# earthspecies/avex

Measured on AMD Instinct MI355X. Metric: clips/s (10 s @ 16 kHz) embedding extraction, BEATs-base, higher is better.
Workload: dtype f16; 1 GPU; BEATs-base (12L/768/3072/12H, 90.7 M params, synthetic weights), batch 256 x 10 s @ 16 kHz per GPU, wav resident in HBM -> mean-pooled 768-d embedding; global_batch=256, samples_per_clip=160000, parallelism=dp1, world_size=1, inputs=avex_amd.synth.noise_clips(seed=0), keyed by global clip index, chunk_clips=256, streams=1, residual_stream=half, layernorm_fold=True

## Files before the change

### avex_amd/csrc/attention16.hip

```cpp
#include <stdlib.h>

#include "common.h"
#include "attention_plan.h"

namespace {

typedef int a3_i32x2 __attribute__((ext_vector_type(2)));
typedef int a3_i32x4 __attribute__((ext_vector_type(4)));
template <int N> struct a3_ic { static constexpr int value = N; };
template <typename T> struct a3_v2;
template <> struct a3_v2<_Float16> { typedef _Float16 type __attribute__((ext_vector_type(2))); };
template <> struct a3_v2<__bf16> { typedef __bf16 type __attribute__((ext_vector_type(2))); };

constexpr int A3_TMAX = 512;
constexpr int A3_KBUF = 32768;
constexpr int A3_HALF = 65536;
constexpr int A3_TPAD = 64;
constexpr int A3_TLD = A3_TPAD + 1040;
constexpr int A3_TAB_OFF = 2 * A3_HALF;
constexpr int A3X_KBUF = 9 * 4096;
constexpr int A3X_HALF = 2 * A3X_KBUF;
constexpr int A3X_KN = 544;
constexpr int A3X_KADD_OFF = 2 * A3X_HALF;
constexpr int A3X_GW_OFF = A3X_KADD_OFF + 2 * A3X_KN * 4;
constexpr int ATT3X_LDS = A3X_GW_OFF + 136 * 4;
constexpr int A3_TAB_BYTES = 4 * A3_TLD * 4;
constexpr int A3_KADD_OFF = A3_TAB_OFF + A3_TAB_BYTES;
constexpr int A3_GW_OFF = A3_KADD_OFF + 2 * A3_TMAX * 4;
constexpr int ATT3_LDS = A3_GW_OFF + 136 * 4;
constexpr float A3_THR = 8.f;
constexpr float A3_SUM_HI = 4096.f;
constexpr float A3_SUM_LO = 0.015625f;

#ifndef A3_KO
#define A3_KO 0
#endif
#ifndef A3_STAMPS
#define A3_STAMPS 0
#endif
#if A3_STAMPS
__device__ unsigned long long g_a3_stamps[3 * 16 * 8 * 16 * 16];
#endif

static __device__ __forceinline__ float a3_rows_sum(float x) {
    const unsigned u = __builtin_bit_cast(unsigned, x);
    const auto r = __builtin_amdgcn_permlane16_swap(u, u, false, false);
    const float y = __builtin_bit_cast(float, (unsigned)r[0]) + __builtin_bit_cast(float, (unsigned)r[1]);
    const unsigned v = __builtin_bit_cast(unsigned, y);
    const auto q = __builtin_amdgcn_permlane32_swap(v, v, false, false);
    return __builtin_bit_cast(float, (unsigned)q[0]) + __builtin_bit_cast(float, (unsigned)q[1]);
}
static __device__ __forceinline__ float a3_rows_max(float x) {
    const unsigned u = __builtin_bit_cast(unsigned, x);
    const auto r = __builtin_amdgcn_permlane16_swap(u, u, false, false);
    const float y = fmaxf(__builtin_bit_cast(float, (unsigned)r[0]), __builtin_bit_cast(float, (unsigned)r[1]));
    const unsigned v = __builtin_bit_cast(unsigned, y);
    const auto q = __builtin_amdgcn_permlane32_swap(v, v, false, false);
    return fmaxf(__builtin_bit_cast(float, (unsigned)q[0]), __builtin_bit_cast(float, (unsigned)q[1]));
}

static __device__ __forceinline__ void a3_dma16(const void* src, const char* lds_dst) {
    const unsigned lds = (unsigned)(__UINTPTR_TYPE__)(__attribute__((address_space(3))) const char*)lds_dst;
    asm volatile("s_mov_b32 m0, %1\n\tglobal_load_lds_dwordx4 %0, off" ::"v"(src), "s"(lds) : "memory");
}

template <typename T, bool BIAS, bool XT = false>
__global__ __launch_bounds__(512) void attention3_kernel(const T* __restrict__ qkv, int Tn, int Tq, int H, int Bc, int per_block,
                                                        const float* __restrict__ bias_tab, const float* __restrict__ grep_w,
                                                        const float* __restrict__ grep_b, const float* __restrict__ grep_a,
                                                        const uint8_t* __restrict__ key_pad, T* __restrict__ out, int q_log2e) {
    extern __shared__ __attribute__((aligned(16))) char smem[];
    typedef typename Half<T>::v8 v8;
    typedef typename Half<T>::v4 v4;
    static_assert(!XT || !BIAS, "the nine-tile last phase takes the bias table's LDS");
    constexpr int NB = 4, NW = 8, NT = 512, NKT = XT ? 9 : 8;
    constexpr int KBUF = XT ? A3X_KBUF : A3_KBUF, HALF = XT ? A3X_HALF : A3_HALF, KN = XT ? A3X_KN : A3_TMAX;
    float* tab = (float*)(smem + A3_TAB_OFF);
    float* kadd = (float*)(smem + (XT ? A3X_KADD_OFF : A3_KADD_OFF));
    T* gwh = (T*)(smem + (XT ? A3X_GW_OFF : A3_GW_OFF));
    float* gwb = (float*)(smem + (XT ? A3X_GW_OFF : A3_GW_OFF) + 512);

    const int tid = threadIdx.x, lane = tid & 63;
    const int wave = __builtin_amdgcn_readfirstlane(tid >> 6);
    const int c = lane & 15, g = lane >> 4;
    const int n_units = Bc * H;
    const int w0 = blockIdx.x * per_block;
    const int w1 = w0 + per_block < n_units ? w0 + per_block : n_units;
    if (w0 >= w1) return;
    const int E = H * 64;
    const int64_t ld = 3 * (int64_t)E;
    const float NEG_INF = -__builtin_inff();
    const int nh = Tn > 256 ? 2 : 1;
    const int np = (w1 - w0) * nh;
    const int nkt = (Tn + 31) >> 5;
    const int Q0 = 64 * wave;
    const bool has_q = Q0 < Tq;

    int h_cur = w0 / Bc, b_cur = w0 - h_cur * Bc;
    int half = 0;
    int h_ld = h_cur, b_ld = b_cur, half_ld = 0;
    int item_par = 0;

    auto dma_piece = [&](int ph, int u) __attribute__((always_inline)) {
        const T* base = qkv + (int64_t)b_ld * Tn * ld + h_ld * 64;
        char* buf = smem + (ph & 1) * HALF;
        int lane = tid & 63;
        asm volatile("" : "+v"(lane));
        const int ri = 4 * wave + u;
        const int kl = 8 * ri + (lane >> 3);
        int key = half_ld * 256 + kl;
        key = key < Tn ? key : Tn - 1;
        const int chunk = (lane & 7) ^ ((kl >> 1) & 7);
        a3_dma16(base + (int64_t)key * ld + E + chunk * 8, buf + ri * 1024);
        int vkey = half_ld * 256 + 8 * ri + ((lane >> 1) & 7);
        vkey = vkey < Tn ? vkey : Tn - 1;
        a3_dma16(base + (int64_t)vkey * ld + 2 * E + 16 * (lane >> 4) + 8 * (lane & 1), buf + KBUF + ri * 1024);
        if (XT && u == 3 && half_ld == nh - 1 && wave < 4) {
            const int rx = 32 + wave;
            const int klx = 8 * rx + (lane >> 3);
            int kx = half_ld * 256 + klx;
            kx = kx < Tn ? kx : Tn - 1;
            a3_dma16(base + (int64_t)kx * ld + E + ((lane & 7) ^ ((klx >> 1) & 7)) * 8, buf + rx * 1024);
            int vx = half_ld * 256 + 8 * rx + ((lane >> 1) & 7);
            vx = vx < Tn ? vx : Tn - 1;
            a3_dma16(base + (int64_t)vx * ld + 2 * E + 16 * (lane >> 4) + 8 * (lane & 1), buf + KBUF + rx * 1024);
        }
    };
    auto dma_advance = [&]() __attribute__((always_inline)) {
        if (++half_ld == nh) { half_ld = 0; if (++b_ld == Bc) { b_ld = 0; ++h_ld; } }
    };
    auto write_kadd = [&](int slot, int b) __attribute__((always_inline)) {
        for (int j = tid; j < KN; j += NT) {
            bool ok = j < Tn;
            if (ok && key_pad) ok = key_pad[(int64_t)b * Tn + j] == 0;
            kadd[slot * KN + j] = ok ? 0.f : NEG_INF;
        }
    };

    v8 qf[NB][2];
    auto load_q = [&](int h, int b) __attribute__((always_inline)) {
        const T* base = qkv + (int64_t)b * Tn * ld + h * 64;
        int lane = tid & 63;
        asm volatile("" : "+v"(lane));
        const int c = lane & 15, g = lane >> 4;
#pragma unroll
        for (int nb = 0; nb < NB; ++nb) {
            int q = Q0 + 16 * nb + c;
            q = q < Tq ? q : Tq - 1;
            const T* src = base + (int64_t)q * ld + 8 * g;
            asm volatile("global_load_dwordx4 %0, %2, off\n\tglobal_load_dwordx4 %1, %2, off offset:64" : "=&v"(qf[nb][0]), "=&v"(qf[nb][1]) : "v"(src) : "memory");
        }
    };
    if (wave >= NW / 2) __builtin_amdgcn_s_setprio(1);
    load_q(h_cur, b_cur);
#pragma unroll
    for (int u = 0; u < 4; ++u) dma_piece(0, u);
    dma_advance();
    write_kadd(0, b_cur);
    if (tid < 64) {
        float a = 0.f, bb = 0.f;
        if (grep_w) {
            a = (grep_w[0 * 64 + tid] + grep_w[1 * 64 + tid]) + (grep_w[2 * 64 + tid] + grep_w[3 * 64 + tid]);
            bb = (grep_w[4 * 64 + tid] + grep_w[5 * 64 + tid]) + (grep_w[6 * 64 + tid] + grep_w[7 * 64 + tid]);
        }
        const float wsc = 8.0f * 0.6931471805599453f;
        const float wa = a * wsc, wb = bb * wsc;
        const T wah = (T)wa, wbh = (T)wb;
        gwh[0 * 64 + tid] = wah; gwh[1 * 64 + tid] = wbh;
        gwh[2 * 64 + tid] = (T)(wa - (float)wah); gwh[3 * 64 + tid] = (T)(wb - (float)wbh);
        if (tid == 0) {
            gwb[0] = grep_w ? (grep_b[0] + grep_b[1]) + (grep_b[2] + grep_b[3]) : 0.f;
            gwb[1] = grep_w ? (grep_b[4] + grep_b[5]) + (grep_b[6] + grep_b[7]) : 0.f;
        }
    }
    if (tid < 4 * A3_TPAD) tab[(tid >> 6) * A3_TLD + (tid & 63)] = 0.f;

    int h_tab = -1;
    f32x2 gm[NB];
    float l_run[NB];
    unsigned long long refm[NB];
    f32x4 o[NB][4];
#pragma unroll
    for (int nb = 0; nb < NB; ++nb) {
        gm[nb] = (f32x2){1.f, 0.f}; l_run[nb] = 0.f; refm[nb] = 0ull;
#pragma unroll
        for (int db = 0; db < 4; ++db) o[nb][db] = (f32x4){0.f, 0.f, 0.f, 0.f};
    }
    const int v_lane = 1024 * (g >> 1) + 128 * (g & 1) + 32 * (c >> 2) + 8 * (c & 3);
    const float cs = q_log2e ? 0.125f : 0.125f * 1.4426950408889634f;

    int n_st = 0;
    auto store_item = [&](int h, int b) __attribute__((always_inline)) {
        n_st = 0;
        if (!has_q) return;
        int lane = tid & 63;
        asm volatile("" : "+v"(lane));
        const int c = lane & 15, g = lane >> 4;
#pragma unroll
        for (int nb = 0; nb < NB; ++nb) n_st += Q0 + 16 * nb < Tq ? 2 : 0;
#pragma unroll
        for (int nb = 0; nb < NB; ++nb) {
            if (Q0 + 16 * nb >= Tq) continue;
            const float l_tot = a3_rows_sum(l_run[nb]);
            const float inv = __builtin_amdgcn_rcpf(l_tot);
            const f32x2 inv2 = {inv, inv};
            typedef typename a3_v2<T>::type v2;
            auto pk = [&](const f32x4 v, int hi) __attribute__((always_inline)) -> unsigned {
                const f32x2 x = (f32x2){v[2 * hi], v[2 * hi + 1]} * inv2;
                const v2 h = {(T)x[0], (T)x[1]};
                unsigned u = __builtin_bit_cast(unsigned, h);
                asm volatile("" : "+v"(u));
                return u;
            };
            int w[2][4];
#pragma unroll
            for (int p = 0; p < 2; ++p) {
                const auto s0 = __builtin_amdgcn_permlane16_swap(pk(o[nb][2 * p], 0), pk(o[nb][2 * p + 1], 0), false, false);
                const auto s1 = __builtin_amdgcn_permlane16_swap(pk(o[nb][2 * p], 1), pk(o[nb][2 * p + 1], 1), false, false);
                w[p][0] = (int)s0[0]; w[p][1] = (int)s1[0]; w[p][2] = (int)s0[1]; w[p][3] = (int)s1[1];
            }
            const int qrow = Q0 + 16 * nb + c;
            T* orow = out + ((int64_t)b * Tn + qrow) * E + h * 64 + 16 * (g & 1) + 8 * (g >> 1);
#pragma unroll
            for (int p = 0; p < 2; ++p) {
                const a3_i32x4 wv = {w[p][0], w[p][1], w[p][2], w[p][3]};
                if (qrow < Tq) *(a3_i32x4*)(orow + 32 * p) = wv;
            }
        }
    };

    for (int ph = 0; ph < np; ++ph) {
        const bool last_half = half == nh - 1;
        const bool more_items = ph + (nh - half) < np;
#define A3_PT(i) if (A3_STAMPS) { __builtin_amdgcn_sched_barrier(0); pt[i] = __builtin_amdgcn_s_memtime(); __builtin_amdgcn_sched_barrier(0); }
        unsigned long long pt[16];
        if (A3_STAMPS) { for (int i = 0; i < 16; ++i) pt[i] = 0; pt[15] = __builtin_amdgcn_s_memrealtime(); }
        A3_PT(0)
        {
            const int nwait = (half == 0 && ph > 0) ? n_st : 0;
            asm volatile("s_cmp_eq_u32 %8, 8\n\ts_cbranch_scc1 1f\n\t"
                         "s_cmp_eq_u32 %8, 6\n\ts_cbranch_scc1 2f\n\t"
                         "s_cmp_eq_u32 %8, 4\n\ts_cbranch_scc1 3f\n\t"
                         "s_cmp_eq_u32 %8, 2\n\ts_cbranch_scc1 4f\n\t"
                         "s_waitcnt vmcnt(0) lgkmcnt(0)\n\ts_branch 5f\n"
                         "1:\n\ts_waitcnt vmcnt(8) lgkmcnt(0)\n\ts_branch 5f\n"
                         "2:\n\ts_waitcnt vmcnt(6) lgkmcnt(0)\n\ts_branch 5f\n"
                         "3:\n\ts_waitcnt vmcnt(4) lgkmcnt(0)\n\ts_branch 5f\n"
                         "4:\n\ts_waitcnt vmcnt(2) lgkmcnt(0)\n"
                         "5:"
                         : "+v"(qf[0][0]), "+v"(qf[0][1]), "+v"(qf[1][0]), "+v"(qf[1][1]), "+v"(qf[2][0]), "+v"(qf[2][1]), "+v"(qf[3][0]), "+v"(qf[3][1])
                         : "s"(nwait)
                         : "scc", "memory");
        }
        __builtin_amdgcn_s_barrier();
        A3_PT(1)
        if (half == 0) {
            if (BIAS && h_cur != h_tab) {
                for (int r = tid; r < 1040; r += NT) {
                    float v = 0.f;
                    if (r < 2 * Tn - 1) v = bias_tab[(int64_t)h_cur * (2 * Tn - 1) + r] * 1.4426950408889634f;
#pragma unroll
                    for (int sft = 0; sft < 4; ++sft)
                        if (r - sft >= 0) tab[sft * A3_TLD + A3_TPAD + (r - sft)] = v;
                }
                h_tab = h_cur;
                __syncthreads();
            }
            if (more_items) {
                int bn = b_cur + 1;
                bn = bn == Bc ? 0 : bn;
                write_kadd(item_par ^ 1, bn);
            }
            const T qs = (T)cs;
#pragma unroll
            for (int nb = 0; nb < NB; ++nb)
#pragma unroll
                for (int s = 0; s < 2; ++s)
#pragma unroll
                    for (int e8 = 0; e8 < 8; ++e8) qf[nb][s][e8] = qf[nb][s][e8] * qs;
            if (grep_w) {
                const v8 gA0 = *(const v8*)(gwh + (c & 3) * 64 + 8 * g), gA1 = *(const v8*)(gwh + (c & 3) * 64 + 32 + 8 * g);
                const float ba = gwb[0], bb = gwb[1], ah = grep_a[h_cur];
#pragma unroll
                for (int nb = 0; nb < NB; ++nb) {
                    f32x4 acc = mfma16(gA0, qf[nb][0], (f32x4){0.f, 0.f, 0.f, 0.f});
                    acc = mfma16(gA1, qf[nb][1], acc);
                    const float sa = (acc[0] + acc[2]) + ba, sb = (acc[1] + acc[3]) + bb;
                    const float ga = __builtin_amdgcn_rcpf(1.f + __expf(-sa)), gb = __builtin_amdgcn_rcpf(1.f + __expf(-sb));
                    gm[nb][0] = ga * (gb * ah - 1.f) + 2.f;
                }
            } else {
#pragma unroll
                for (int nb = 0; nb < NB; ++nb) gm[nb][0] = 1.f;
            }
        }
        const bool do_dma = ph + 1 < np;
        int dma_done = 0;
        A3_PT(2)
        if (has_q) {
            const char* Kb = smem + (ph & 1) * HALF;
            const float* kad = kadd + item_par * KN + half * 256 + 4 * g;
            const int kt_lim = (XT && last_half) ? 9 : 8;
            int kt_end = nkt - half * 8 < kt_lim ? nkt - half * 8 : kt_lim;
            const char* kp[2];
#pragma unroll
            for (int s = 0; s < 2; ++s) kp[s] = Kb + c * 128 + (((4 * s + g) ^ ((c >> 1) & 7)) << 4);
            const int e0 = 4 * g - (Q0 + c) + (Tn - 1) + 256 * half;
            const float* tp = tab + (e0 & 3) * A3_TLD + A3_TPAD + (e0 & ~3);
            const unsigned vaddr = (unsigned)(__UINTPTR_TYPE__)(__attribute__((address_space(3))) const char*)(Kb + KBUF + v_lane);

            v8 kf[2][2];
#pragma unroll
            for (int s = 0; s < 2; ++s)
#pragma unroll
                for (int kb = 0; kb < 2; ++kb) kf[s][kb] = *(const v8*)(kp[s] + 2048 * kb);
            f32x4 run[5];
            f32x4 Sq[NB][2];
            auto masked_at = [&](int ktl) __attribute__((always_inline)) { return key_pad != nullptr || (half * 8 + ktl) * 32 + 32 > Tn; };
            auto acc_start = [&](int nb, int kb, const f32x4 t4) __attribute__((always_inline)) {
                const f32x2 ta = {t4[0], t4[1]}, tb = {t4[2], t4[3]};
                f32x2 ea, eb;
                asm("v_pk_fma_f32 %0, %1, %2, %1 op_sel:[0,0,1] op_sel_hi:[0,1,1] neg_lo:[0,0,1] neg_hi:[0,0,1]" : "=v"(ea) : "v"(gm[nb]), "v"(ta));
                asm("v_pk_fma_f32 %0, %1, %2, %1 op_sel:[0,0,1] op_sel_hi:[0,1,1] neg_lo:[0,0,1] neg_hi:[0,0,1]" : "=v"(eb) : "v"(gm[nb]), "v"(tb));
                Sq[nb][kb] = (f32x4){ea[0], ea[1], eb[0], eb[1]};
            };
            auto acc_plain = [&](int nb) __attribute__((always_inline)) {
                const float nm = -gm[nb][1];
                Sq[nb][0] = (f32x4){nm, nm, nm, nm};
                Sq[nb][1] = (f32x4){nm, nm, nm, nm};
            };
            auto mask_acc = [&](int ktl) __attribute__((always_inline)) {
                const f32x4 k0 = *(const f32x4*)(kad + 32 * ktl), k1 = *(const f32x4*)(kad + 32 * ktl + 16);
#pragma unroll
                for (int nb = 0; nb < NB; ++nb) { Sq[nb][0] += k0; Sq[nb][1] += k1; }
            };
            if (BIAS) {
#pragma unroll
                for (int w = -3; w <= 1; ++w) run[w + 3] = *(const f32x4*)(tp + 16 * w);
#pragma unroll
                for (int nb = 0; nb < NB; ++nb)
#pragma unroll
                    for (int kb = 0; kb < 2; ++kb) acc_start(nb, kb, run[kb - nb + 3]);
            } else {
#pragma unroll
                for (int nb = 0; nb < NB; ++nb) acc_plain(nb);
            }
            if (masked_at(0)) mask_acc(0);
#define A3_FENCE() do { if (!(A3_KO & 32)) __builtin_amdgcn_sched_barrier(0); } while (0)
            auto tile = [&](auto KT) __attribute__((always_inline)) {
                constexpr int kt = decltype(KT)::value;
                typedef typename a3_v2<T>::type v2;
                a3_i32x2 vt[2][4];
                f32x2 pp[NB][4];
                unsigned pfw[NB][4];
                f32x2 lsa[NB], lsb[NB];
                float sum[NB];
                unsigned long long badm[NB];
                auto E = [&](int nb, int i) __attribute__((always_inline)) {
                    const int kb = i >> 1, r = 2 * (i & 1);
                    if (A3_KO & 2) { pp[nb][i] = (f32x2){Sq[nb][kb][r], Sq[nb][kb][r + 1]}; return; }
                    float x0 = Sq[nb][kb][r], x1 = Sq[nb][kb][r + 1];
                    asm volatile("" : "+v"(x0), "+v"(x1));
                    Sq[nb][kb][r] = x0; Sq[nb][kb][r + 1] = x1;
                    pp[nb][i] = (f32x2){__builtin_amdgcn_exp2f(x0), __builtin_amdgcn_exp2f(x1)};
                };
                auto cvt2 = [&](const f32x2 x) __attribute__((always_inline)) -> unsigned {
                    const v2 h = {(T)x[0], (T)x[1]};
                    unsigned u = __builtin_bit_cast(unsigned, h);
                    asm volatile("" : "+v"(u));
                    return u;
                };
                auto X = [&](int nb, int i) __attribute__((always_inline)) {
                    if (i == 0) { pfw[nb][0] = cvt2(pp[nb][0]); pfw[nb][1] = cvt2(pp[nb][1]); lsa[nb] = pp[nb][0] + pp[nb][1]; }
                    if (i == 1) { pfw[nb][2] = cvt2(pp[nb][2]); pfw[nb][3] = cvt2(pp[nb][3]); lsb[nb] = pp[nb][2] + pp[nb][3]; }
                    if (i == 2) { lsa[nb] += lsb[nb]; sum[nb] = hsum2(lsa[nb]); }
                    if (i == 3) {
                        badm[nb] = __builtin_amdgcn_ballot_w64(!(sum[nb] < A3_SUM_HI)) | (__builtin_amdgcn_ballot_w64(!(sum[nb] >= A3_SUM_LO)) & ~refm[nb]);
                    }
                };
                auto redo = [&](int nb) __attribute__((always_inline)) {
                    float mx = fmaxf(fmaxf(fmaxf(Sq[nb][0][0], Sq[nb][0][1]), fmaxf(Sq[nb][0][2], Sq[nb][0][3])),
                                     fmaxf(fmaxf(Sq[nb][1][0], Sq[nb][1][1]), fmaxf(Sq[nb][1][2], Sq[nb][1][3])));
                    mx = a3_rows_max(mx);
                    const bool rs = (refm[nb] >> lane) & 1ull;
                    const bool need = rs ? mx > A3_THR : mx != NEG_INF;
                    const float d = need ? mx : 0.f;
                    const float alpha = (need && rs) ? __builtin_amdgcn_exp2f(-d) : 1.f;
                    refm[nb] |= __builtin_amdgcn_ballot_w64(need);
                    gm[nb][1] += d;
                    l_run[nb] *= alpha;
#pragma unroll
                    for (int db = 0; db < 4; ++db) o[nb][db] *= alpha;
                    f32x2 ls = {0.f, 0.f};
#pragma unroll
                    for (int i = 0; i < 4; ++i) {
                        const int kb = i >> 1, r = 2 * (i & 1);
                        const f32x2 q2 = {__builtin_amdgcn_exp2f(Sq[nb][kb][r] - d), __builtin_amdgcn_exp2f(Sq[nb][kb][r + 1] - d)};
                        ls += q2;
                        const v2 h = {(T)q2[0], (T)q2[1]};
                        pfw[nb][i] = __builtin_bit_cast(unsigned, h);
                    }
                    sum[nb] = hsum2(ls);
                };
                auto check = [&](int nb) __attribute__((always_inline)) {
                    if (A3_KO & 1) { }
                    else if (__builtin_expect(badm[nb] != 0ull, 0)) redo(nb);
                    else refm[nb] = ~0ull;
                    l_run[nb] += sum[nb];
                };
                auto pfrag = [&](int nb) __attribute__((always_inline)) -> v8 {
                    typedef unsigned a3_u32x4 __attribute__((ext_vector_type(4)));
                    const a3_u32x4 w = {pfw[nb][0], pfw[nb][1], pfw[nb][2], pfw[nb][3]};
                    return __builtin_bit_cast(v8, w);
                };
                auto acc_next = [&](int j) __attribute__((always_inline)) {
                    if (kt + 1 >= NKT) return;
                    const int nn = j >> 1, kb = j & 1;
                    if ((A3_KO & 16) || !BIAS) { if (kb == 0) acc_plain(nn); }
                    else acc_start(nn, kb, run[(2 * (kt + 1) + kb - nn + 3) % 5]);
                };
#define A3_TS(i) if (A3_STAMPS == 2 && (kt == 6 || kt == 1)) { __builtin_amdgcn_sched_barrier(0); ts[i] = __builtin_amdgcn_s_memtime(); __builtin_amdgcn_sched_barrier(0); }
                unsigned long long ts[12];
                A3_TS(0)
#pragma unroll
                for (int i = 0; i < 4; ++i) {
                    const int s = i >> 1, kb = i & 1;
                    if (!(A3_KO & 4)) Sq[0][kb] = mfma16(kf[s][kb], qf[0][s], Sq[0][kb]);
                    A3_FENCE();
                }
                if (kt < 4 && do_dma) { dma_piece(ph + 1, kt); dma_done = kt + 1; A3_FENCE(); }
                {
#define A3_TR(dst, OFF) asm volatile("ds_read_b64_tr_b16 %0, %1 offset:%2" : "=v"(dst) : "v"(vaddr), "n"(OFF))
                    A3_TR(vt[0][0], 4096 * kt + 0);    A3_TR(vt[1][0], 4096 * kt + 2048 + 0);
                    A3_TR(vt[0][1], 4096 * kt + 256);  A3_TR(vt[1][1], 4096 * kt + 2048 + 256);
                    A3_TR(vt[0][2], 4096 * kt + 512);  A3_TR(vt[1][2], 4096 * kt + 2048 + 512);
                    A3_TR(vt[0][3], 4096 * kt + 768);  A3_TR(vt[1][3], 4096 * kt + 2048 + 768);
#undef A3_TR
                    if (BIAS && kt + 1 < NKT) {
                        run[(2 * kt + 5) % 5] = *(const f32x4*)(tp + 16 * (2 * kt + 2));
                        run[(2 * kt + 6) % 5] = *(const f32x4*)(tp + 16 * (2 * kt + 3));
                    }
                    A3_FENCE();
                }
                A3_TS(1)
#pragma unroll
                for (int nb = 1; nb < NB; ++nb) {
#pragma unroll
                    for (int i = 0; i < 4; ++i) {
                        const int s = i >> 1, kb = i & 1;
                        if (!(A3_KO & 4)) Sq[nb][kb] = mfma16(kf[s][kb], qf[nb][s], Sq[nb][kb]);
                        A3_FENCE();
                        E(nb - 1, i);
                        if (nb >= 2) X(nb - 2, i);
                        A3_FENCE();
                    }
                    A3_TS(1 + nb)
                }
                check(0);
                A3_FENCE();
                asm volatile("s_waitcnt lgkmcnt(0)"
                             : "+v"(vt[0][0]), "+v"(vt[0][1]), "+v"(vt[0][2]), "+v"(vt[0][3]), "+v"(vt[1][0]), "+v"(vt[1][1]), "+v"(vt[1][2]), "+v"(vt[1][3]));
                v8 vf[4];
#pragma unroll
                for (int db = 0; db < 4; ++db) {
                    const v4 lo = __builtin_bit_cast(v4, vt[0][db]), hi = __builtin_bit_cast(v4, vt[1][db]);
                    vf[db] = __builtin_shufflevector(lo, hi, 0, 1, 2, 3, 4, 5, 6, 7);
                }
                if (kt + 1 < NKT) {
#pragma unroll
                    for (int s = 0; s < 2; ++s)
#pragma unroll
                        for (int kb = 0; kb < 2; ++kb) kf[s][kb] = *(const v8*)(kp[s] + 4096 * (kt + 1) + 2048 * kb);
                }
                A3_FENCE();
                A3_TS(5)
                {
                    const v8 pf = pfrag(0);
#pragma unroll
                    for (int db = 0; db < 4; ++db) {
                        if (!(A3_KO & 8)) o[0][db] = mfma16(vf[db], pf, o[0][db]);
                        A3_FENCE();
                        E(3, db);
                        X(2, db);
                        A3_FENCE();
                    }
                }
                check(1);
                A3_FENCE();
                A3_TS(6)
                {
                    const v8 pf = pfrag(1);
#pragma unroll
                    for (int db = 0; db < 4; ++db) {
                        if (!(A3_KO & 8)) o[1][db] = mfma16(vf[db], pf, o[1][db]);
                        A3_FENCE();
                        X(3, db);
                        if (db >= 2) acc_next(db - 2);
                        A3_FENCE();
                    }
                }
                check(2);
                A3_FENCE();
                A3_TS(7)
                {
                    const v8 pf = pfrag(2);
#pragma unroll
                    for (int db = 0; db < 4; ++db) {
                        if (!(A3_KO & 8)) o[2][db] = mfma16(vf[db], pf, o[2][db]);
                        A3_FENCE();
                        if (db < 3) { acc_next(2 + db); A3_FENCE(); }
                    }
                }
                check(3);
                A3_FENCE();
                A3_TS(8)
                {
                    const v8 pf = pfrag(3);
#pragma unroll
                    for (int db = 0; db < 4; ++db) {
                        if (!(A3_KO & 8)) o[3][db] = mfma16(vf[db], pf, o[3][db]);
                        A3_FENCE();
                        if (db < 3) { acc_next(5 + db); A3_FENCE(); }
                    }
                }
                A3_TS(9)
                if (kt + 1 < NKT && masked_at(kt + 1)) mask_acc(kt + 1);
#if A3_STAMPS == 2
                if ((kt == 6 || kt == 1) && blockIdx.x < 16 && lane == 0 && ph < 16) {
                    unsigned long long* d = g_a3_stamps + (((size_t)(16 + blockIdx.x) * 8 + wave) * 16 + ph) * 16;
                    if (kt == 6) d += 16 * 8 * 16 * 16;
                    for (int i = 0; i < 10; ++i) d[i] = ts[i];
                }
#endif
#undef A3_TS
            };
            A3_PT(3)
            if (0 < kt_end) tile(a3_ic<0>{});
            A3_PT(4)
            if (1 < kt_end) tile(a3_ic<1>{});
            A3_PT(5)
            if (2 < kt_end) tile(a3_ic<2>{});
            A3_PT(6)
            if (3 < kt_end) tile(a3_ic<3>{});
            A3_PT(7)
            if (4 < kt_end) tile(a3_ic<4>{});
            A3_PT(8)
            if (5 < kt_end) tile(a3_ic<5>{});
            A3_PT(9)
            if (6 < kt_end) tile(a3_ic<6>{});
            A3_PT(10)
            if (7 < kt_end) tile(a3_ic<7>{});
            if constexpr (XT) { if (8 < kt_end) tile(a3_ic<8>{}); }
#undef A3_FENCE
        }
        if (do_dma) {
            for (int u = dma_done; u < 4; ++u) dma_piece(ph + 1, u);
            dma_advance();
        }
        A3_PT(11)
        if (last_half) {
            int hn = h_cur, bn = b_cur + 1;
            if (bn == Bc) { bn = 0; ++hn; }
            if (more_items) load_q(hn, bn);
            A3_PT(13)
            store_item(h_cur, b_cur);
            A3_PT(14)
            item_par ^= 1;
            h_cur = hn; b_cur = bn;
#pragma unroll
            for (int nb = 0; nb < NB; ++nb) {
                gm[nb][1] = 0.f; l_run[nb] = 0.f; refm[nb] = 0ull;
#pragma unroll
                for (int db = 0; db < 4; ++db) o[nb][db] = (f32x4){0.f, 0.f, 0.f, 0.f};
            }
        }
        half = last_half ? 0 : half + 1;
        A3_PT(12)
#undef A3_PT
#if A3_STAMPS
        if (blockIdx.x < 16 && lane == 0 && ph < 16) {
            unsigned long long* d = g_a3_stamps + (((size_t)blockIdx.x * 8 + wave) * 16 + ph) * 16;
            for (int i = 0; i < 16; ++i) d[i] = pt[i];
        }
#endif
    }
}

static_assert(A3_TMAX == avx::ATT_PLAN_TMAX && ATT3_LDS == avx::ATT_PLAN_LDS3 && ATT3X_LDS == avx::ATT_PLAN_LDS3X, "attention_plan.h plans for these kernels");

template <typename T>
int launch3(const void* qkv, int B, int Tn, int H, const float* bias_tab, const float* grep_w, const float* grep_b, const float* grep_a,
            const uint8_t* key_pad, void* out, int q_log2e, const avx::AttPlan& p, hipStream_t s) {
    const int Tq = Tn < A3_TMAX ? Tn : A3_TMAX;
#define AVX_ATT3(BIAS, XT) do { AVX_ENSURE_LDS((attention3_kernel<T, BIAS, XT>), p.lds); \
        hipLaunchKernelGGL((attention3_kernel<T, BIAS, XT>), dim3(p.grid), dim3(p.block), p.lds, s, (const T*)qkv, Tn, Tq, H, B, p.per_block, bias_tab, grep_w, grep_b, \
                           grep_a, key_pad, (T*)out, q_log2e); } while (0)
    if (p.k_xt) AVX_ATT3(false, true); else if (p.k_bias) AVX_ATT3(true, false); else AVX_ATT3(false, false);
#undef AVX_ATT3
    AVX_LAUNCH_CHECK();
    return AVEXHIP_OK;
}

}

namespace avx {

int attention16(const void* qkv, int B, int T, int H, const float* bias_tab, const float* grep_w, const float* grep_b, const float* grep_a,
                const uint8_t* key_pad, void* out, int dtype, int q_log2e, const AttPlan& p, hipStream_t s) {
    AVX_REQUIRE(T > 0 && (T <= A3_TMAX || (T <= A3_TMAX + 32 && !bias_tab)), "attention16: T=%d tokens (1..512, or up to 544 without a bias table)", T);
    AVX_REQUIRE((int64_t)B * H < (1ll << 31), "attention16: too many (clip, head) items");
    if (dtype == AVEXHIP_F16) return launch3<_Float16>(qkv, B, T, H, bias_tab, grep_w, grep_b, grep_a, key_pad, out, q_log2e, p, s);
    if (dtype == AVEXHIP_BF16) return launch3<__bf16>(qkv, B, T, H, bias_tab, grep_w, grep_b, grep_a, key_pad, out, q_log2e, p, s);
    avexhip_set_error("attention16: unknown dtype %d", dtype);
    return AVEXHIP_ERR_INVALID;
}

}
```

Measured before the change: 10250 clips/s.

## Defer output store of finished attention item to after next barrier for half the waves

When an item finishes and more items follow, waves in the first half defer the output store and accumulator reset until after the next phase's barrier. This lets the next Q load and the cross-wave barrier proceed without waiting on the store. The other half still store immediately, which staggers the write traffic. The waitcnt asm is factored into a macro, and deferred phases wait with vmcnt(8). This adds register pressure from holding the accumulators across the barrier, and it changes the ordering of the vmcnt accounting.

```diff
diff --git a/avex_amd/csrc/attention16.hip b/avex_amd/csrc/attention16.hip
--- a/avex_amd/csrc/attention16.hip
+++ b/avex_amd/csrc/attention16.hip
@@ -229,6 +229,28 @@
         }
     };
 
+    auto reset_item = [&]() __attribute__((always_inline)) {
+#pragma unroll
+        for (int nb = 0; nb < NB; ++nb) {
+            gm[nb][1] = 0.f; l_run[nb] = 0.f; refm[nb] = 0ull;
+#pragma unroll
+            for (int db = 0; db < 4; ++db) o[nb][db] = (f32x4){0.f, 0.f, 0.f, 0.f};
+        }
+    };
+    int deferred = 0;
+    int h_prev = 0, b_prev = 0;
+#define A3_WAIT(n, ...) asm volatile("s_cmp_eq_u32 %[nw], 8\n\ts_cbranch_scc1 1f\n\t"                 \
+                                     "s_cmp_eq_u32 %[nw], 6\n\ts_cbranch_scc1 2f\n\t"                 \
+                                     "s_cmp_eq_u32 %[nw], 4\n\ts_cbranch_scc1 3f\n\t"                 \
+                                     "s_cmp_eq_u32 %[nw], 2\n\ts_cbranch_scc1 4f\n\t"                 \
+                                     "s_waitcnt vmcnt(0) lgkmcnt(0)\n\ts_branch 5f\n"                 \
+                                     "1:\n\ts_waitcnt vmcnt(8) lgkmcnt(0)\n\ts_branch 5f\n"           \
+                                     "2:\n\ts_waitcnt vmcnt(6) lgkmcnt(0)\n\ts_branch 5f\n"           \
+                                     "3:\n\ts_waitcnt vmcnt(4) lgkmcnt(0)\n\ts_branch 5f\n"           \
+                                     "4:\n\ts_waitcnt vmcnt(2) lgkmcnt(0)\n"                          \
+                                     "5:"                                                             \
+                                     : __VA_ARGS__ : [nw] "s"(n) : "scc", "memory")
+
     for (int ph = 0; ph < np; ++ph) {
         const bool last_half = half == nh - 1;
         const bool more_items = ph + (nh - half) < np;
@@ -236,24 +258,33 @@
         unsigned long long pt[16];
         if (A3_STAMPS) { for (int i = 0; i < 16; ++i) pt[i] = 0; pt[15] = __builtin_amdgcn_s_memrealtime(); }
         A3_PT(0)
+#if A3_STAMPS
+        bool stamps_written = false;
+        auto write_stamps = [&]() __attribute__((always_inline)) {
+            if (blockIdx.x < 16 && lane == 0 && ph < 16) {
+                unsigned long long* d = g_a3_stamps + (((size_t)blockIdx.x * 8 + wave) * 16 + ph) * 16;
+                for (int i = 0; i < 16; ++i) d[i] = pt[i];
+            }
+            stamps_written = true;
+        };
+#endif
+        {
+            const int npre = deferred ? 8 : (half == 0 && ph > 0) ? n_st : 0;
+            A3_WAIT(npre, );
+        }
+        __builtin_amdgcn_s_barrier();
+        A3_PT(1)
+        if (deferred) {
+            A3_PT(13)
+            store_item(h_prev, b_prev);
+            reset_item();
+            A3_PT(14)
+            deferred = 0;
+        }
         {
             const int nwait = (half == 0 && ph > 0) ? n_st : 0;
-            asm volatile("s_cmp_eq_u32 %8, 8\n\ts_cbranch_scc1 1f\n\t"
-                         "s_cmp_eq_u32 %8, 6\n\ts_cbranch_scc1 2f\n\t"
-                         "s_cmp_eq_u32 %8, 4\n\ts_cbranch_scc1 3f\n\t"
-                         "s_cmp_eq_u32 %8, 2\n\ts_cbranch_scc1 4f\n\t"
-                         "s_waitcnt vmcnt(0) lgkmcnt(0)\n\ts_branch 5f\n"
-                         "1:\n\ts_waitcnt vmcnt(8) lgkmcnt(0)\n\ts_branch 5f\n"
-                         "2:\n\ts_waitcnt vmcnt(6) lgkmcnt(0)\n\ts_branch 5f\n"
-                         "3:\n\ts_waitcnt vmcnt(4) lgkmcnt(0)\n\ts_branch 5f\n"
-                         "4:\n\ts_waitcnt vmcnt(2) lgkmcnt(0)\n"
-                         "5:"
-                         : "+v"(qf[0][0]), "+v"(qf[0][1]), "+v"(qf[1][0]), "+v"(qf[1][1]), "+v"(qf[2][0]), "+v"(qf[2][1]), "+v"(qf[3][0]), "+v"(qf[3][1])
-                         : "s"(nwait)
-                         : "scc", "memory");
-        }
-        __builtin_amdgcn_s_barrier();
-        A3_PT(1)
+            A3_WAIT(nwait, "+v"(qf[0][0]), "+v"(qf[0][1]), "+v"(qf[1][0]), "+v"(qf[1][1]), "+v"(qf[2][0]), "+v"(qf[2][1]), "+v"(qf[3][0]), "+v"(qf[3][1]));
+        }
         if (half == 0) {
             if (BIAS && h_cur != h_tab) {
                 for (int r = tid; r < 1040; r += NT) {
@@ -561,28 +592,28 @@
         if (last_half) {
             int hn = h_cur, bn = b_cur + 1;
             if (bn == Bc) { bn = 0; ++hn; }
+#if A3_STAMPS
+            if (more_items && wave < NW / 2) { A3_PT(12) write_stamps(); }
+#endif
             if (more_items) load_q(hn, bn);
-            A3_PT(13)
-            store_item(h_cur, b_cur);
-            A3_PT(14)
+            if (more_items && wave < NW / 2) {
+                deferred = 1;
+                h_prev = h_cur; b_prev = b_cur;
+            } else {
+                A3_PT(13)
+                store_item(h_cur, b_cur);
+                reset_item();
+                A3_PT(14)
+            }
             item_par ^= 1;
             h_cur = hn; b_cur = bn;
-#pragma unroll
-            for (int nb = 0; nb < NB; ++nb) {
-                gm[nb][1] = 0.f; l_run[nb] = 0.f; refm[nb] = 0ull;
-#pragma unroll
-                for (int db = 0; db < 4; ++db) o[nb][db] = (f32x4){0.f, 0.f, 0.f, 0.f};
-            }
         }
         half = last_half ? 0 : half + 1;
-        A3_PT(12)
+#if A3_STAMPS
+        if (!stamps_written) { A3_PT(12) write_stamps(); }
+#endif
 #undef A3_PT
-#if A3_STAMPS
-        if (blockIdx.x < 16 && lane == 0 && ph < 16) {
-            unsigned long long* d = g_a3_stamps + (((size_t)blockIdx.x * 8 + wave) * 16 + ph) * 16;
-            for (int i = 0; i < 16; ++i) d[i] = pt[i];
-        }
-#endif
+#undef A3_WAIT
     }
 }
 
```

Result: no change. 10270 clips/s (median of 6 runs) (+0.2%).
